# JacobYoung115/VisualSLAM

Hardware: AMD Instinct MI355X
Metric: frames/sec @1080p (Harris + DoG keypoint detection) (higher is better)
Workload: dtype u8

## Files before the change

### visualslam_amd/csrc/diff_taps.gen.h

```cpp
#pragma once
#include <cstdint>

namespace vslam {
namespace dtaps {

constexpr int OCT_LO = 1, OCT_HI = 3;

template <int O, int L>
struct Lvl;

template <>
struct Lvl<1, 0> {
    static constexpr int n = 19, form = 0, nd = 18;
    static constexpr uint16_t w[n] = {1, 1, 3, 6, 9, 15, 20, 27, 30, 32, 30, 27, 20, 15, 9, 6, 3, 1, 1};
    static constexpr int16_t de[nd] = {-10, -8, -7, -6, -5, -4, -3, -2, -1, 0, 1, 2, 3, 4, 5, 6, 7, 9};
    static constexpr int16_t dc[nd] = {-1, -2, -3, -3, -6, -5, -7, -3, -2, 2, 3, 7, 5, 6, 3, 3, 2, 1};
};

template <>
struct Lvl<1, 1> {
    static constexpr int n = 23, form = 0, nd = 22;
    static constexpr uint16_t w[n] = {1, 1, 2, 4, 5, 9, 12, 15, 19, 23, 24, 26, 24, 23, 19, 15, 12, 9, 5, 4, 2, 1, 1};
    static constexpr int16_t de[nd] = {-12, -10, -9, -8, -7, -6, -5, -4, -3, -2, -1, 0, 1, 2, 3, 4, 5, 6, 7, 8, 9, 11};
    static constexpr int16_t dc[nd] = {-1, -1, -2, -1, -4, -3, -3, -4, -4, -1, -2, 2, 1, 4, 4, 3, 3, 4, 1, 2, 1, 1};
};

template <>
struct Lvl<1, 2> {
    static constexpr int n = 29, form = 0, nd = 26;
    static constexpr uint16_t w[n] = {1, 0, 2, 2, 3, 4, 6, 7, 10, 13, 15, 17, 18, 20, 20, 20, 18, 17, 15, 13, 10, 7, 6, 4, 3, 2, 2, 0, 1};
    static constexpr int16_t de[nd] = {-15, -14, -13, -11, -10, -9, -8, -7, -6, -5, -4, -3, -2, 1, 2, 3, 4, 5, 6, 7, 8, 9, 10, 12, 13, 14};
    static constexpr int16_t dc[nd] = {-1, 1, -2, -1, -1, -2, -1, -3, -3, -2, -2, -1, -2, 2, 1, 2, 2, 3, 3, 1, 2, 1, 1, 2, -1, 1};
};

template <>
struct Lvl<1, 3> {
    static constexpr int n = 37, form = 1, nd = 24;
    static constexpr uint16_t w[n] = {1, 0, 1, 1, 1, 2, 3, 4, 4, 6, 8, 8, 11, 11, 14, 14, 15, 16, 16, 16, 15, 14, 14, 11, 11, 8, 8, 6, 4, 4, 3, 2, 1, 1, 1, 0, 1};
    static constexpr int16_t de[nd] = {-19, -18, -17, -14, -13, -12, -10, -9, -7, -5, -3, -2, 1, 2, 4, 6, 8, 9, 11, 12, 13, 16, 17, 18};
    static constexpr int16_t dc[nd] = {-1, 1, -1, -1, -1, -1, -2, -2, -3, -3, -1, -1, 1, 1, 3, 3, 2, 2, 1, 1, 1, 1, -1, 1};
};

template <>
struct Lvl<1, 4> {
    static constexpr int n = 45, form = 1, nd = 36;
    static constexpr uint16_t w[n] = {1, 0, 1, 0, 2, 1, 2, 2, 3, 3, 4, 5, 6, 7, 8, 9, 9, 11, 11, 12, 12, 13, 12, 13, 12, 12, 11, 11, 9, 9, 8, 7, 6, 5, 4, 3, 3, 2, 2, 1, 2, 0, 1, 0, 1};
    static constexpr int16_t de[nd] = {-23, -22, -21, -20, -19, -18, -17, -15, -13, -12, -11, -10, -9, -8, -6, -4, -2, -1, 0, 1, 3, 5, 7, 8, 9, 10, 11, 12, 14, 16, 17, 18, 19, 20, 21, 22};
    static constexpr int16_t dc[nd] = {-1, 1, -1, 1, -2, 1, -1, -1, -1, -1, -1, -1, -1, -1, -2, -1, -1, 1, -1, 1, 1, 2, 1, 1, 1, 1, 1, 1, 1, 1, -1, 2, -1, 1, -1, 1};
};

template <>
struct Lvl<1, 5> {
    static constexpr int n = 57, form = 1, nd = 28;
    static constexpr uint16_t w[n] = {1, 0, 0, 1, 0, 1, 1, 1, 2, 2, 2, 2, 3, 3, 4, 5, 5, 5, 7, 6, 8, 8, 8, 9, 9, 10, 10, 10, 10, 10, 10, 10, 9, 9, 8, 8, 8, 6, 7, 5, 5, 5, 4, 3, 3, 2, 2, 2, 2, 1, 1, 1, 0, 1, 0, 0, 1};
    static constexpr int16_t de[nd] = {-29, -28, -26, -25, -24, -21, -17, -15, -14, -11, -10, -9, -6, -4, 3, 5, 8, 9, 10, 13, 14, 16, 20, 23, 24, 25, 27, 28};
    static constexpr int16_t dc[nd] = {-1, 1, -1, 1, -1, -1, -1, -1, -1, -2, 1, -2, -1, -1, 1, 1, 2, -1, 2, 1, 1, 1, 1, 1, -1, 1, -1, 1};
};

template <>
struct Lvl<2, 0> {
    static constexpr int n = 37, form = 1, nd = 24;
    static constexpr uint16_t w[n] = {1, 0, 1, 1, 1, 2, 3, 4, 4, 6, 8, 8, 11, 11, 14, 14, 15, 16, 16, 16, 15, 14, 14, 11, 11, 8, 8, 6, 4, 4, 3, 2, 1, 1, 1, 0, 1};
    static constexpr int16_t de[nd] = {-19, -18, -17, -14, -13, -12, -10, -9, -7, -5, -3, -2, 1, 2, 4, 6, 8, 9, 11, 12, 13, 16, 17, 18};
    static constexpr int16_t dc[nd] = {-1, 1, -1, -1, -1, -1, -2, -2, -3, -3, -1, -1, 1, 1, 3, 3, 2, 2, 1, 1, 1, 1, -1, 1};
};

template <>
struct Lvl<2, 1> {
    static constexpr int n = 45, form = 1, nd = 36;
    static constexpr uint16_t w[n] = {1, 0, 1, 0, 2, 1, 2, 2, 3, 3, 4, 5, 6, 7, 8, 9, 9, 11, 11, 12, 12, 13, 12, 13, 12, 12, 11, 11, 9, 9, 8, 7, 6, 5, 4, 3, 3, 2, 2, 1, 2, 0, 1, 0, 1};
    static constexpr int16_t de[nd] = {-23, -22, -21, -20, -19, -18, -17, -15, -13, -12, -11, -10, -9, -8, -6, -4, -2, -1, 0, 1, 3, 5, 7, 8, 9, 10, 11, 12, 14, 16, 17, 18, 19, 20, 21, 22};
    static constexpr int16_t dc[nd] = {-1, 1, -1, 1, -2, 1, -1, -1, -1, -1, -1, -1, -1, -1, -2, -1, -1, 1, -1, 1, 1, 2, 1, 1, 1, 1, 1, 1, 1, 1, -1, 2, -1, 1, -1, 1};
};

template <>
struct Lvl<2, 2> {
    static constexpr int n = 57, form = 1, nd = 28;
    static constexpr uint16_t w[n] = {1, 0, 0, 1, 0, 1, 1, 1, 2, 2, 2, 2, 3, 3, 4, 5, 5, 5, 7, 6, 8, 8, 8, 9, 9, 10, 10, 10, 10, 10, 10, 10, 9, 9, 8, 8, 8, 6, 7, 5, 5, 5, 4, 3, 3, 2, 2, 2, 2, 1, 1, 1, 0, 1, 0, 0, 1};
    static constexpr int16_t de[nd] = {-29, -28, -26, -25, -24, -21, -17, -15, -14, -11, -10, -9, -6, -4, 3, 5, 8, 9, 10, 13, 14, 16, 20, 23, 24, 25, 27, 28};
    static constexpr int16_t dc[nd] = {-1, 1, -1, 1, -1, -1, -1, -1, -1, -2, 1, -2, -1, -1, 1, 1, 2, -1, 2, 1, 1, 1, 1, 1, -1, 1, -1, 1};
};

template <>
struct Lvl<2, 3> {
    static constexpr int n = 71, form = 1, nd = 34;
    static constexpr uint16_t w[n] = {1, 0, 0, 1, 0, 0, 1, 1, 1, 1, 1, 1, 2, 2, 2, 2, 3, 3, 3, 4, 4, 4, 5, 5, 6, 5, 7, 6, 7, 7, 8, 7, 8, 8, 8, 8, 8, 8, 8, 7, 8, 7, 7, 6, 7, 5, 6, 5, 5, 4, 4, 4, 3, 3, 3, 2, 2, 2, 2, 1, 1, 1, 1, 1, 1, 0, 0, 1, 0, 0, 1};
    static constexpr int16_t de[nd] = {-36, -35, -33, -32, -30, -24, -20, -17, -14, -12, -11, -10, -9, -8, -6, -5, -4, 3, 4, 5, 7, 8, 9, 10, 11, 13, 16, 19, 23, 29, 31, 32, 34, 35};
    static constexpr int16_t dc[nd] = {-1, 1, -1, 1, -1, -1, -1, -1, -1, -1, 1, -2, 1, -1, -1, 1, -1, 1, -1, 1, 1, -1, 2, -1, 1, 1, 1, 1, 1, 1, -1, 1, -1, 1};
};

template <>
struct Lvl<2, 4> {
    static constexpr int n = 89, form = 1, nd = 44;
    static constexpr uint16_t w[n] = {1, 0, 0, 0, 1, 0, 0, 1, 0, 1, 1, 0, 1, 1, 1, 2, 1, 2, 1, 2, 2, 3, 2, 3, 3, 3, 3, 4, 4, 4, 4, 5, 5, 5, 5, 5, 6, 6, 6, 6, 6, 6, 6, 7, 6, 7, 6, 6, 6, 6, 6, 6, 6, 5, 5, 5, 5, 5, 4, 4, 4, 4, 3, 3, 3, 3, 2, 3, 2, 2, 1, 2, 1, 2, 1, 1, 1, 0, 1, 1, 0, 1, 0, 0, 1, 0, 0, 0, 1};
    static constexpr int16_t de[nd] = {-45, -44, -41, -40, -38, -37, -36, -34, -33, -30, -29, -28, -27, -26, -24, -23, -22, -18, -14, -9, -2, -1, 0, 1, 8, 13, 17, 21, 22, 23, 25, 26, 27, 28, 29, 32, 33, 35, 36, 37, 39, 40, 43, 44};
    static constexpr int16_t dc[nd] = {-1, 1, -1, 1, -1, 1, -1, 1, -1, -1, 1, -1, 1, -1, -1, 1, -1, -1, -1, -1, -1, 1, -1, 1, 1, 1, 1, 1, -1, 1, 1, -1, 1, -1, 1, 1, -1, 1, -1, 1, -1, 1, -1, 1};
};

template <>
struct Lvl<2, 5> {
    static constexpr int n = 111, form = 1, nd = 56;
    static constexpr uint16_t w[n] = {1, 0, 0, 0, 0, 1, 0, 0, 1, 0, 0, 1, 0, 1, 1, 0, 1, 1, 1, 1, 1, 1, 2, 1, 2, 1, 2, 2, 2, 3, 2, 2, 3, 3, 3, 3, 3, 4, 3, 4, 4, 4, 4, 4, 4, 5, 4, 5, 5, 5, 5, 4, 5, 5, 5, 6, 5, 5, 5, 4, 5, 5, 5, 5, 4, 5, 4, 4, 4, 4, 4, 4, 3, 4, 3, 3, 3, 3, 3, 2, 2, 3, 2, 2, 2, 1, 2, 1, 2, 1, 1, 1, 1, 1, 1, 0, 1, 1, 0, 1, 0, 0, 1, 0, 0, 1, 0, 0, 0, 0, 1};
    static constexpr int16_t de[nd] = {-56, -55, -51, -50, -48, -47, -45, -44, -43, -41, -40, -34, -33, -32, -31, -30, -27, -26, -24, -19, -18, -17, -11, -10, -9, -5, -4, -1, 0, 3, 4, 8, 9, 10, 16, 17, 18, 23, 25, 26, 29, 30, 31, 32, 33, 39, 40, 42, 43, 44, 46, 47, 49, 50, 54, 55};
    static constexpr int16_t dc[nd] = {-1, 1, -1, 1, -1, 1, -1, 1, -1, 1, -1, -1, 1, -1, 1, -1, -1, 1, -1, -1, 1, -1, -1, 1, -1, 1, -1, -1, 1, 1, -1, 1, -1, 1, 1, -1, 1, 1, -1, 1, 1, -1, 1, -1, 1, 1, -1, 1, -1, 1, -1, 1, -1, 1, -1, 1};
};

template <>
struct Lvl<3, 0> {
    static constexpr int n = 71, form = 1, nd = 34;
    static constexpr uint16_t w[n] = {1, 0, 0, 1, 0, 0, 1, 1, 1, 1, 1, 1, 2, 2, 2, 2, 3, 3, 3, 4, 4, 4, 5, 5, 6, 5, 7, 6, 7, 7, 8, 7, 8, 8, 8, 8, 8, 8, 8, 7, 8, 7, 7, 6, 7, 5, 6, 5, 5, 4, 4, 4, 3, 3, 3, 2, 2, 2, 2, 1, 1, 1, 1, 1, 1, 0, 0, 1, 0, 0, 1};
    static constexpr int16_t de[nd] = {-36, -35, -33, -32, -30, -24, -20, -17, -14, -12, -11, -10, -9, -8, -6, -5, -4, 3, 4, 5, 7, 8, 9, 10, 11, 13, 16, 19, 23, 29, 31, 32, 34, 35};
    static constexpr int16_t dc[nd] = {-1, 1, -1, 1, -1, -1, -1, -1, -1, -1, 1, -2, 1, -1, -1, 1, -1, 1, -1, 1, 1, -1, 2, -1, 1, 1, 1, 1, 1, 1, -1, 1, -1, 1};
};

template <>
struct Lvl<3, 1> {
    static constexpr int n = 89, form = 1, nd = 44;
    static constexpr uint16_t w[n] = {1, 0, 0, 0, 1, 0, 0, 1, 0, 1, 1, 0, 1, 1, 1, 2, 1, 2, 1, 2, 2, 3, 2, 3, 3, 3, 3, 4, 4, 4, 4, 5, 5, 5, 5, 5, 6, 6, 6, 6, 6, 6, 6, 7, 6, 7, 6, 6, 6, 6, 6, 6, 6, 5, 5, 5, 5, 5, 4, 4, 4, 4, 3, 3, 3, 3, 2, 3, 2, 2, 1, 2, 1, 2, 1, 1, 1, 0, 1, 1, 0, 1, 0, 0, 1, 0, 0, 0, 1};
    static constexpr int16_t de[nd] = {-45, -44, -41, -40, -38, -37, -36, -34, -33, -30, -29, -28, -27, -26, -24, -23, -22, -18, -14, -9, -2, -1, 0, 1, 8, 13, 17, 21, 22, 23, 25, 26, 27, 28, 29, 32, 33, 35, 36, 37, 39, 40, 43, 44};
    static constexpr int16_t dc[nd] = {-1, 1, -1, 1, -1, 1, -1, 1, -1, -1, 1, -1, 1, -1, -1, 1, -1, -1, -1, -1, -1, 1, -1, 1, 1, 1, 1, 1, -1, 1, 1, -1, 1, -1, 1, 1, -1, 1, -1, 1, -1, 1, -1, 1};
};

template <>
struct Lvl<3, 2> {
    static constexpr int n = 111, form = 1, nd = 56;
    static constexpr uint16_t w[n] = {1, 0, 0, 0, 0, 1, 0, 0, 1, 0, 0, 1, 0, 1, 1, 0, 1, 1, 1, 1, 1, 1, 2, 1, 2, 1, 2, 2, 2, 3, 2, 2, 3, 3, 3, 3, 3, 4, 3, 4, 4, 4, 4, 4, 4, 5, 4, 5, 5, 5, 5, 4, 5, 5, 5, 6, 5, 5, 5, 4, 5, 5, 5, 5, 4, 5, 4, 4, 4, 4, 4, 4, 3, 4, 3, 3, 3, 3, 3, 2, 2, 3, 2, 2, 2, 1, 2, 1, 2, 1, 1, 1, 1, 1, 1, 0, 1, 1, 0, 1, 0, 0, 1, 0, 0, 1, 0, 0, 0, 0, 1};
    static constexpr int16_t de[nd] = {-56, -55, -51, -50, -48, -47, -45, -44, -43, -41, -40, -34, -33, -32, -31, -30, -27, -26, -24, -19, -18, -17, -11, -10, -9, -5, -4, -1, 0, 3, 4, 8, 9, 10, 16, 17, 18, 23, 25, 26, 29, 30, 31, 32, 33, 39, 40, 42, 43, 44, 46, 47, 49, 50, 54, 55};
    static constexpr int16_t dc[nd] = {-1, 1, -1, 1, -1, 1, -1, 1, -1, 1, -1, -1, 1, -1, 1, -1, -1, 1, -1, -1, 1, -1, -1, 1, -1, 1, -1, -1, 1, 1, -1, 1, -1, 1, 1, -1, 1, 1, -1, 1, 1, -1, 1, -1, 1, 1, -1, 1, -1, 1, -1, 1, -1, 1, -1, 1};
};

template <>
struct Lvl<3, 3> {
    static constexpr int n = 141, form = 1, nd = 64;
    static constexpr uint16_t w[n] = {1, 0, 0, 0, 0, 0, 0, 1, 0, 0, 0, 1, 0, 0, 1, 0, 0, 1, 0, 1, 1, 0, 1, 1, 0, 1, 1, 1, 1, 1, 1, 2, 1, 1, 2, 1, 2, 2, 2, 2, 2, 2, 2, 2, 3, 2, 3, 2, 3, 3, 3, 3, 3, 3, 4, 3, 3, 4, 4, 3, 4, 4, 3, 4, 4, 4, 4, 4, 4, 4, 4, 4, 4, 4, 4, 4, 4, 4, 3, 4, 4, 3, 4, 4, 3, 3, 4, 3, 3, 3, 3, 3, 3, 2, 3, 2, 3, 2, 2, 2, 2, 2, 2, 2, 2, 1, 2, 1, 1, 2, 1, 1, 1, 1, 1, 1, 0, 1, 1, 0, 1, 1, 0, 1, 0, 0, 1, 0, 0, 1, 0, 0, 0, 1, 0, 0, 0, 0, 0, 0, 1};
    static constexpr int16_t de[nd] = {-71, -70, -64, -63, -60, -59, -57, -56, -54, -53, -52, -50, -49, -47, -46, -40, -39, -37, -36, -35, -27, -26, -25, -24, -23, -17, -16, -14, -12, -11, -9, -8, 7, 8, 10, 11, 13, 15, 16, 22, 23, 24, 25, 26, 34, 35, 36, 38, 39, 45, 46, 48, 49, 51, 52, 53, 55, 56, 58, 59, 62, 63, 69, 70};
    static constexpr int16_t dc[nd] = {-1, 1, -1, 1, -1, 1, -1, 1, -1, 1, -1, 1, -1, 1, -1, -1, 1, -1, 1, -1, -1, 1, -1, 1, -1, -1, 1, -1, 1, -1, 1, -1, 1, -1, 1, -1, 1, -1, 1, 1, -1, 1, -1, 1, 1, -1, 1, -1, 1, 1, -1, 1, -1, 1, -1, 1, -1, 1, -1, 1, -1, 1, -1, 1};
};

template <>
struct Lvl<3, 4> {
    static constexpr int n = 177, form = 1, nd = 80;
    static constexpr uint16_t w[n] = {1, 0, 0, 0, 0, 0, 0, 0, 0, 1, 0, 0, 0, 0, 1, 0, 0, 0, 1, 0, 0, 1, 0, 1, 0, 0, 1, 0, 1, 1, 0, 1, 1, 0, 1, 1, 1, 1, 1, 1, 1, 1, 1, 1, 1, 2, 1, 2, 1, 2, 1, 2, 1, 2, 2, 2, 2, 2, 2, 2, 2, 2, 3, 2, 3, 2, 2, 3, 3, 2, 3, 3, 3, 2, 3, 3, 3, 3, 3, 3, 3, 4, 3, 3, 3, 3, 3, 3, 4, 3, 3, 3, 3, 3, 3, 4, 3, 3, 3, 3, 3, 3, 3, 2, 3, 3, 3, 2, 3, 3, 2, 2, 3, 2, 3, 2, 2, 2, 2, 2, 2, 2, 2, 2, 1, 2, 1, 2, 1, 2, 1, 2, 1, 1, 1, 1, 1, 1, 1, 1, 1, 1, 1, 0, 1, 1, 0, 1, 1, 0, 1, 0, 0, 1, 0, 1, 0, 0, 1, 0, 0, 0, 1, 0, 0, 0, 0, 1, 0, 0, 0, 0, 0, 0, 0, 0, 1};
    static constexpr int16_t de[nd] = {-89, -88, -80, -79, -75, -74, -71, -70, -68, -67, -66, -65, -63, -62, -61, -59, -58, -56, -55, -44, -43, -42, -41, -40, -39, -38, -37, -36, -27, -26, -25, -24, -22, -20, -19, -16, -15, -8, -7, -1, 0, 6, 7, 14, 15, 18, 19, 21, 23, 24, 25, 26, 35, 36, 37, 38, 39, 40, 41, 42, 43, 54, 55, 57, 58, 60, 61, 62, 64, 65, 66, 67, 69, 70, 73, 74, 78, 79, 87, 88};
    static constexpr int16_t dc[nd] = {-1, 1, -1, 1, -1, 1, -1, 1, -1, 1, -1, 1, -1, 1, -1, 1, -1, 1, -1, -1, 1, -1, 1, -1, 1, -1, 1, -1, -1, 1, -1, 1, -1, 1, -1, 1, -1, -1, 1, -1, 1, -1, 1, 1, -1, 1, -1, 1, -1, 1, -1, 1, 1, -1, 1, -1, 1, -1, 1, -1, 1, 1, -1, 1, -1, 1, -1, 1, -1, 1, -1, 1, -1, 1, -1, 1, -1, 1, -1, 1};
};

template <>
struct Lvl<3, 5> {
    static constexpr int n = 223, form = 1, nd = 116;
    static constexpr uint16_t w[n] = {1, 0, 0, 0, 0, 0, 0, 0, 0, 0, 0, 1, 0, 0, 0, 0, 0, 0, 1, 0, 0, 0, 0, 1, 0, 0, 0, 1, 0, 0, 1, 0, 1, 0, 0, 1, 0, 1, 0, 1, 0, 1, 0, 1, 1, 0, 1, 1, 1, 0, 1, 1, 1, 1, 1, 1, 1, 1, 1, 1, 1, 1, 2, 1, 1, 1, 2, 1, 2, 1, 2, 1, 2, 1, 2, 2, 1, 2, 2, 2, 2, 2, 2, 2, 2, 2, 2, 2, 2, 2, 2, 3, 2, 2, 3, 2, 2, 3, 2, 2, 3, 2, 3, 2, 3, 2, 3, 2, 3, 2, 3, 2, 3, 2, 3, 2, 3, 2, 3, 2, 3, 2, 3, 2, 2, 3, 2, 2, 3, 2, 2, 3, 2, 2, 2, 2, 2, 2, 2, 2, 2, 2, 2, 2, 2, 2, 1, 2, 2, 1, 2, 1, 2, 1, 2, 1, 2, 1, 1, 1, 2, 1, 1, 1, 1, 1, 1, 1, 1, 1, 1, 1, 1, 0, 1, 1, 1, 0, 1, 1, 0, 1, 0, 1, 0, 1, 0, 1, 0, 0, 1, 0, 1, 0, 0, 1, 0, 0, 0, 1, 0, 0, 0, 0, 1, 0, 0, 0, 0, 0, 0, 1, 0, 0, 0, 0, 0, 0, 0, 0, 0, 0, 1};
    static constexpr int16_t de[nd] = {-112, -111, -101, -100, -94, -93, -89, -88, -85, -84, -82, -81, -80, -79, -77, -76, -75, -74, -73, -72, -71, -70, -69, -67, -66, -63, -62, -50, -49, -46, -45, -44, -43, -42, -41, -40, -39, -38, -36, -35, -21, -20, -18, -17, -15, -14, -12, -11, -10, -9, -8, -7, -6, -5, -4, -3, -2, -1, 0, 1, 2, 3, 4, 5, 6, 7, 8, 9, 10, 11, 13, 14, 16, 17, 19, 20, 34, 35, 37, 38, 39, 40, 41, 42, 43, 44, 45, 48, 49, 61, 62, 65, 66, 68, 69, 70, 71, 72, 73, 74, 75, 76, 78, 79, 80, 81, 83, 84, 87, 88, 92, 93, 99, 100, 110, 111};
    static constexpr int16_t dc[nd] = {-1, 1, -1, 1, -1, 1, -1, 1, -1, 1, -1, 1, -1, 1, -1, 1, -1, 1, -1, 1, -1, 1, -1, 1, -1, 1, -1, -1, 1, -1, 1, -1, 1, -1, 1, -1, 1, -1, 1, -1, -1, 1, -1, 1, -1, 1, -1, 1, -1, 1, -1, 1, -1, 1, -1, 1, -1, 1, -1, 1, -1, 1, -1, 1, -1, 1, -1, 1, -1, 1, -1, 1, -1, 1, -1, 1, 1, -1, 1, -1, 1, -1, 1, -1, 1, -1, 1, -1, 1, 1, -1, 1, -1, 1, -1, 1, -1, 1, -1, 1, -1, 1, -1, 1, -1, 1, -1, 1, -1, 1, -1, 1, -1, 1, -1, 1};
};

}
}
```

### visualslam_amd/csrc/kernels_hdiff.hip.h

```cpp
#pragma once
#include <hip/hip_runtime.h>

#include <utility>
#include <vector>

#include "diff_taps.gen.h"
#include "kernels_strip.hip.h"
#include "vslam_internal.h"

namespace vslam {

constexpr int HD_J = 16;
constexpr int HD_PAD = 2;

typedef float hd_f2 __attribute__((ext_vector_type(2)));

template <class F, int... I>
__device__ __forceinline__ void hd_for_impl(F&& f, std::integer_sequence<int, I...>) {
    (f(std::integral_constant<int, I>{}), ...);
}
template <int N, class F>
__device__ __forceinline__ void hd_for(F&& f) {
    hd_for_impl(f, std::make_integer_sequence<int, N>{});
}

__host__ __device__ constexpr int hd_phys(int c) { return c + (c >> 4) * HD_PAD; }

template <class LV>
__host__ __device__ constexpr int hd_w(int k) { return k >= 0 && k < LV::n ? (int)LV::w[k] : 0; }

template <class LV>
__host__ __device__ constexpr int hd_coef(int e) {
    if (LV::form == 1) {
        for (int i = 0; i < LV::nd; ++i)
            if (LV::de[i] == e) return LV::dc[i];
        return 0;
    }
    return hd_w<LV>(e + LV::n / 2);
}

template <int O>
struct HdGeom {
    static constexpr int nmax = dtaps::Lvl<O, 5>::n;
    static constexpr int rmax = nmax / 2;
    static constexpr int HL = (rmax + 2 + 15) & ~15;
    static_assert(dtaps::Lvl<O, 0>::n <= nmax && dtaps::Lvl<O, 4>::n <= nmax, "level 5 is the widest");
};

__host__ __device__ inline int hd_pw(int cols, int HL, int rmax) {
    const int ccount = HL + 16 * ((cols + HD_J - 1) / HD_J) + rmax;
    return (ccount + 1 + 15) / 16 * (16 + HD_PAD);
}

template <class LV, int HL>
__device__ __forceinline__ void hd_level(const hd_f2* __restrict__ lane, hd_f2 (&acc)[HD_J]) {
    constexpr int n = LV::n, r = n / 2;
    constexpr bool DIFF = LV::form == 1;
    constexpr int lo = DIFF ? -r - 1 : -r, hi = HD_J - 1 + r;
    constexpr int t0 = (HL + lo) & ~1, Q = (HL + hi - t0) / 2 + 1;
    hd_f2 seed = {0.f, 0.f};
    hd_for<HD_J>([&](auto j) { acc[decltype(j)::value] = hd_f2{0.f, 0.f}; });
    hd_for<Q>([&](auto q) {
        constexpr int t = t0 + 2 * decltype(q)::value;
        const float4 v = *reinterpret_cast<const float4*>(lane + hd_phys(t));
        const hd_f2 hv[2] = {hd_f2{v.x, v.y}, hd_f2{v.z, v.w}};
        hd_for<2>([&](auto b) {
            constexpr int x = t + decltype(b)::value - HL;
            if constexpr (DIFF) {
                constexpr int wk = hd_w<LV>(x + 1 + r);
                if constexpr (wk != 0) seed = __builtin_elementwise_fma(hd_f2((float)wk), hv[decltype(b)::value], seed);
            }
            hd_for<HD_J>([&](auto j) {
                constexpr int c = hd_coef<LV>(x - decltype(j)::value);
                if constexpr (c != 0)
                    acc[decltype(j)::value] = __builtin_elementwise_fma(hd_f2((float)c), hv[decltype(b)::value], acc[decltype(j)::value]);
            });
        });
    });
    if constexpr (DIFF) {
        acc[0] += seed;
        hd_for<HD_J - 1>([&](auto j) { acc[decltype(j)::value + 1] += acc[decltype(j)::value]; });
    }
}

template <int O>
__global__ __launch_bounds__(256) void k_gauss_h_diff(const uint16_t* __restrict__ h, size_t hframe, uint8_t* __restrict__ oct_out,
                                                       size_t pframe, int rows, int cols, int pitch, int npairs, int pw,
                                                       uint8_t* __restrict__ next_base, size_t nframe, int nrows, int ncols, int npitch) {
    using G = HdGeom<O>;
    extern __shared__ __attribute__((aligned(16))) uint32_t smem[];
    hd_f2* hp = reinterpret_cast<hd_f2*>(smem);
    const int tid = threadIdx.x;
    const int y0 = blockIdx.y * 2 * npairs;
    const size_t P = (size_t)rows * pitch;
    uint8_t* out = oct_out + blockIdx.z * pframe;
    const int ncs = (cols + HD_J - 1) / HD_J;
    const int ccount = G::HL + HD_J * ncs + G::rmax;
    const int n8 = cols >> 3, nb = ccount - 8 * n8;
    const bool active = tid < npairs * ncs;
    const int ip = tid / ncs, is = tid - ip * ncs;
    const hd_f2* lane = hp + ip * pw + is * (HD_J + HD_PAD);
    const int n8d = max(n8, 1);
    const int i_p0 = tid / n8d, i_k0 = tid - i_p0 * n8d, i_dp = 256 / n8d, i_dk = 256 - i_dp * n8d;
    const int b_p0 = tid / nb, b_i0 = tid - b_p0 * nb, b_dp = 256 / nb, b_di = 256 - b_dp * nb;
    uint32_t prev_e[2][4], prev_o[2][4];

    hd_for<VSLAM_NUM_LEVELS>([&](auto lc) {
        constexpr int L = decltype(lc)::value;
        const uint16_t* hl = h + blockIdx.z * hframe + (size_t)L * P;
        __syncthreads();
        for (int it = tid, p = i_p0, k = i_k0; it < npairs * n8; it += 256, p += i_dp, k += i_dk) {
            if (k >= n8) k -= n8, ++p;
            const uint4 a = *reinterpret_cast<const uint4*>(hl + (size_t)min(y0 + 2 * p, rows - 1) * pitch + 8 * k);
            const uint4 b = *reinterpret_cast<const uint4*>(hl + (size_t)min(y0 + 2 * p + 1, rows - 1) * pitch + 8 * k);
            float4* q = reinterpret_cast<float4*>(hp + p * pw + hd_phys(G::HL + 8 * k));
            const uint32_t av[4] = {a.x, a.y, a.z, a.w}, bv[4] = {b.x, b.y, b.z, b.w};
#pragma unroll
            for (int i = 0; i < 4; ++i)
                q[i] = make_float4((float)(av[i] & 0xffffu), (float)(bv[i] & 0xffffu), (float)(av[i] >> 16), (float)(bv[i] >> 16));
        }
        for (int it = tid, p = b_p0, i = b_i0; it < npairs * nb; it += 256, p += b_dp, i += b_di) {
            if (i >= nb) i -= nb, ++p;
            const int c = i < G::HL ? i : 8 * n8 + i;
            const int x = reflect101(c - G::HL, cols);
            const uint16_t* ra = hl + (size_t)min(y0 + 2 * p, rows - 1) * pitch;
            const uint16_t* rb = hl + (size_t)min(y0 + 2 * p + 1, rows - 1) * pitch;
            hp[p * pw + hd_phys(c)] = hd_f2{(float)ra[x], (float)rb[x]};
        }
        __syncthreads();
        if (active) {
            hd_f2 acc[HD_J];
            hd_level<dtaps::Lvl<O, L>, G::HL>(lane, acc);
            const int x = HD_J * is;
            hd_for<2>([&](auto rc) {
                constexpr int rho = decltype(rc)::value;
                const int y = y0 + 2 * ip + rho;
                uint32_t u[HD_J], g[4], d[4];
                hd_for<HD_J>([&](auto j) { u[decltype(j)::value] = (uint32_t)acc[decltype(j)::value][rho]; });
#pragma unroll
                for (int hw = 0; hw < 4; ++hw) {
                    const uint32_t e = __builtin_amdgcn_perm(u[4 * hw + 2], u[4 * hw + 0], 0x0c060c02);
                    const uint32_t o = __builtin_amdgcn_perm(u[4 * hw + 3], u[4 * hw + 1], 0x0c060c02);
                    g[hw] = __builtin_amdgcn_perm(o, e, 0x06020400);
                    if constexpr (L > 0)
                        d[hw] = __builtin_amdgcn_perm(pk_sub_sat_u16(o, prev_o[rho][hw]), pk_sub_sat_u16(e, prev_e[rho][hw]), 0x06020400);
                    prev_e[rho][hw] = e;
                    prev_o[rho][hw] = o;
                }
                if (y < rows) {
                    const size_t off = (size_t)y * pitch + x;
                    *reinterpret_cast<uint4*>(out + (size_t)L * P + off) = make_uint4(g[0], g[1], g[2], g[3]);
                    if constexpr (L > 0)
                        *reinterpret_cast<uint4*>(out + (size_t)(VSLAM_NUM_LEVELS + L - 1) * P + off) = make_uint4(d[0], d[1], d[2], d[3]);
                    if constexpr (L == 3 && rho == 0)
                        if (next_base && (y >> 1) < nrows && (x >> 1) < ncols)
                            *reinterpret_cast<uint2*>(next_base + blockIdx.z * nframe + (size_t)(y >> 1) * npitch + (x >> 1)) =
                                make_uint2(__builtin_amdgcn_perm(g[1], g[0], 0x06040200), __builtin_amdgcn_perm(g[3], g[2], 0x06040200));
                }
            });
        }
    });
}

template <int O, int L>
static bool hd_level_matches(const std::vector<uint16_t>& t) {
    using LV = dtaps::Lvl<O, L>;
    if ((int)t.size() != LV::n) return false;
    for (int k = 0; k < LV::n; ++k)
        if (t[k] != LV::w[k]) return false;
    std::vector<int> off, coef;
    if (diff_form(t.data(), LV::n, off, coef) != LV::form) return false;
    if (LV::form == 1) {
        if ((int)off.size() != LV::nd) return false;
        for (int i = 0; i < LV::nd; ++i)
            if (off[i] != LV::de[i] || coef[i] != LV::dc[i]) return false;
    }
    return true;
}
template <int O>
static bool hd_octave_matches(const std::vector<uint16_t> (&taps)[6]) {
    return hd_level_matches<O, 0>(taps[0]) && hd_level_matches<O, 1>(taps[1]) && hd_level_matches<O, 2>(taps[2]) &&
           hd_level_matches<O, 3>(taps[3]) && hd_level_matches<O, 4>(taps[4]) && hd_level_matches<O, 5>(taps[5]);
}

}
```

### visualslam_amd/csrc/vslam_internal.h

```cpp
#pragma once
#include <cstddef>
#include <cstdint>
#include <vector>

#include "../../include/vslam.h"

#define VSLAM_MAX_KSIZE 4095

namespace vslam {
int gauss_ksize_u8(double sigma);
bool gauss_taps_q8(int n, double sigma, uint16_t* taps);
bool gauss_taps_q8_trimmed(int n, double sigma, std::vector<uint16_t>& out);
int gauss_ksize_f32(double sigma);
bool gauss_kernel_f32(int n, double sigma, std::vector<float>& out);
double sigma_at(double sigma0, int octave, int level);
int auto_num_octaves(int rows, int cols);
void half_size(int rows, int cols, int* r, int* c);
void extrema_lattice(int rows, int cols, int window, int* lr, int* lc);
int make_layout(const vslam_params* p, vslam_batch_layout* L);
int diff_form(const uint16_t* w, int n, std::vector<int>& off, std::vector<int>& coef);
}

extern "C" int vslam_diff_form_q8(const uint16_t* taps, int n, int* offsets, int* coeffs, int cap, int* nnz);
```

### visualslam_amd/csrc/vslam_params.cpp

```cpp
#include <cmath>
#include <cstdio>
#include <cstring>
#include <vector>

#include "../../include/vslam.h"
#include "vslam_internal.h"

namespace vslam {

static inline long cv_round(double v) { return std::lrint(v); }

int gauss_ksize_u8(double sigma) { return (int)cv_round(sigma * 3 * 2 + 1) | 1; }

static void gauss_kernel_f64(int n, double sigma, std::vector<double>& kf) {
    kf.assign((size_t)n, 0.0);
    const int half = (n - 1) / 2;
    static const double k3[] = {0.25, 0.5, 0.25};
    static const double k5[] = {0.0625, 0.25, 0.375, 0.25, 0.0625};
    static const double k7[] = {0.03125, 0.109375, 0.21875, 0.28125, 0.21875, 0.109375, 0.03125};
    if (sigma <= 0 && n == 1) {
        kf[0] = 1.0;
    } else if (sigma <= 0 && n == 3) {
        kf.assign(k3, k3 + 3);
    } else if (sigma <= 0 && n == 5) {
        kf.assign(k5, k5 + 5);
    } else if (sigma <= 0 && n == 7) {
        kf.assign(k7, k7 + 7);
    } else {
        const double s = sigma > 0 ? sigma : std::fma((double)n, 0.15, 0.35);
        const double scale = -0.125 / (s * s);
        double sum = 0.0;
        for (int i = 0, x = 1 - n; i < half; ++i, x += 2) {
            kf[i] = std::exp((double)(x * x) * scale);
            sum += kf[i];
        }
        sum = sum * 2.0 + 1.0;
        const double inv = 1.0 / sum;
        for (int i = 0; i < half; ++i) kf[n - 1 - i] = kf[i] = kf[i] * inv;
        kf[half] = inv;
    }
}

int gauss_ksize_f32(double sigma) { return (int)cv_round(sigma * 4 * 2 + 1) | 1; }

bool gauss_kernel_f32(int n, double sigma, std::vector<float>& out) {
    if (n <= 0 || (n & 1) == 0 || n > (1 << 20)) return false;
    std::vector<double> kf;
    gauss_kernel_f64(n, sigma, kf);
    out.resize((size_t)n);
    for (int i = 0; i < n; ++i) out[(size_t)i] = (float)kf[(size_t)i];
    return true;
}

bool gauss_taps_q8(int n, double sigma, uint16_t* taps) {
    if (n <= 0 || (n & 1) == 0 || n > VSLAM_MAX_KSIZE) return false;
    std::vector<double> kf;
    gauss_kernel_f64(n, sigma, kf);
    double err = 0.0;
    long acc = 0;
    for (int i = 0; i < n / 2; ++i) {
        const double adj = kf[i] * 256.0 + err;
        const long q = cv_round(adj);
        err = adj - (double)q;
        taps[i] = taps[n - 1 - i] = (uint16_t)q;
        acc += q;
    }
    taps[n / 2] = (uint16_t)(256 - 2 * acc);
    return true;
}

bool gauss_taps_q8_trimmed(int n, double sigma, std::vector<uint16_t>& out) {
    std::vector<uint16_t> t((size_t)(n > 0 ? n : 0));
    if (!gauss_taps_q8(n, sigma, t.data())) return false;
    int z = 0;
    while (2 * z + 1 < n && t[z] == 0 && t[n - 1 - z] == 0) ++z;
    out.assign(t.begin() + z, t.end() - z);
    return true;
}

static constexpr long DIFF_HMAX = 255 * 256 + 128;

int diff_form(const uint16_t* w, int n, std::vector<int>& off, std::vector<int>& coef) {
    off.clear(), coef.clear();
    if (!w || n <= 0 || (n & 1) == 0) return -1;
    const int r = n / 2;
    long l1 = 0;
    for (int e = -r - 1; e <= r; ++e) {
        const int k = e + r;
        const int d = (k >= 0 ? (int)w[k] : 0) - (k + 1 < n ? (int)w[k + 1] : 0);
        if (d) off.push_back(e), coef.push_back(d), l1 += d < 0 ? -d : d;
    }
    if (l1 * DIFF_HMAX >= (1L << 24)) return 0;
    return (double)off.size() * 2.32 * 1.15 <= (double)(n + 1) / 2 * 4.27 ? 1 : 0;
}

double sigma_at(double sigma0, int octave, int level) {
    const double k = std::pow(2.0f, 1.0f / (double)3);
    return std::pow(2, octave) * sigma0 * std::pow(k, level);
}

int auto_num_octaves(int rows, int cols) {
    const int m = rows < cols ? rows : cols;
    return (int)std::floor(std::log2((double)m)) - 4;
}

void half_size(int rows, int cols, int* r, int* c) {
    *r = (int)cv_round(rows * 0.5);
    *c = (int)cv_round(cols * 0.5);
}

void extrema_lattice(int rows, int cols, int window, int* lr, int* lc) {
    const int pad = (window - 1) / 2;
    *lr = rows > pad ? (rows - pad + window - 1) / window : 0;
    *lc = cols > pad ? (cols - pad + window - 1) / window : 0;
}

int make_layout(const vslam_params* p, vslam_batch_layout* L) {
    if (!p || !L || p->rows <= 0 || p->cols <= 0 || p->n_octaves < 0 || p->n_octaves > VSLAM_MAX_OCTAVES)
        return VSLAM_ERR_INVALID;
    if (p->n_octaves > 0 && (!(p->sigma0 > 0) || p->extrema_window < 3 || (p->extrema_window & 1) == 0))
        return VSLAM_ERR_INVALID;
    if (p->n_octaves > 0 && p->extrema_dense && (p->extrema_window != 3 || p->localize || p->orient)) return VSLAM_ERR_INVALID;
    std::memset(L, 0, sizeof(*L));
    L->n_octaves = p->n_octaves;
    int r = p->rows * 2, c = p->cols * 2;
    size_t off = 0, woff = 0, sum_p = 0;
    for (int o = 0; o < p->n_octaves; ++o) {
        if (r <= 0 || c <= 0) return VSLAM_ERR_INVALID;
        L->rows[o] = r;
        L->cols[o] = c;
        if (p->extrema_dense)
            L->lat_rows[o] = r, L->lat_cols[o] = c;
        else
            extrema_lattice(r, c, p->extrema_window, &L->lat_rows[o], &L->lat_cols[o]);
        L->lat_words[o] = (L->lat_cols[o] + 63) / 64;
        L->octave_offset[o] = off;
        L->bits_offset[o] = woff;
        L->pitch[o] = (c + 15) & ~15;
        const size_t P = (size_t)r * c;
        sum_p += P;
        off += (VSLAM_NUM_LEVELS + VSLAM_NUM_DOGS) * ((size_t)r * L->pitch[o]);
        woff += (size_t)3 * L->lat_rows[o] * L->lat_words[o];
        half_size(r, c, &r, &c);
    }
    L->pyramid_frame_bytes = (off + 255) & ~(size_t)255;
    L->bits_frame_words = woff;
    const size_t N = (size_t)p->rows * p->cols;
    L->algorithmic_bytes_harris = 6 * N;
    L->algorithmic_bytes_dog = N + 11 * sum_p;
    return VSLAM_OK;
}

}

extern "C" {

int vslam_version(void) { return VSLAM_VERSION; }

const char* vslam_status_string(int s) {
    switch (s) {
        case VSLAM_OK: return "ok";
        case VSLAM_ERR_INVALID: return "invalid argument";
        case VSLAM_ERR_HIP: return "HIP runtime error";
        case VSLAM_ERR_NOMEM: return "out of memory";
        case VSLAM_ERR_UNSUPPORTED: return "unsupported parameter combination";
        case VSLAM_ERR_RANGE: return "octave/level out of range";
        default: return "unknown status";
    }
}

int vslam_gauss_ksize_u8(double sigma) { return vslam::gauss_ksize_u8(sigma); }

int vslam_gauss_taps_q8(int n, double sigma, uint16_t* taps) {
    if (!taps) return VSLAM_ERR_INVALID;
    return vslam::gauss_taps_q8(n, sigma, taps) ? VSLAM_OK : VSLAM_ERR_INVALID;
}

double vslam_sigma_at(double sigma0, int octave, int level) { return vslam::sigma_at(sigma0, octave, level); }

int vslam_diff_form_q8(const uint16_t* taps, int n, int* offsets, int* coeffs, int cap, int* nnz) {
    std::vector<int> off, coef;
    const int form = vslam::diff_form(taps, n, off, coef);
    if (form < 0 || !nnz || (int)off.size() > cap || (!off.empty() && (!offsets || !coeffs))) return -1;
    *nnz = (int)off.size();
    for (size_t i = 0; i < off.size(); ++i) offsets[i] = off[i], coeffs[i] = coef[i];
    return form;
}
int vslam_auto_num_octaves(int rows, int cols) { return vslam::auto_num_octaves(rows, cols); }

void vslam_half_size(int rows, int cols, int* out_rows, int* out_cols) {
    vslam::half_size(rows, cols, out_rows, out_cols);
}

void vslam_extrema_lattice(int rows, int cols, int window, int* lat_rows, int* lat_cols) {
    vslam::extrema_lattice(rows, cols, window, lat_rows, lat_cols);
}

void vslam_params_default(vslam_params* p, int rows, int cols) {
    if (!p) return;
    p->rows = rows;
    p->cols = cols;
    p->n_octaves = 4;
    p->sigma0 = 1.6;
    p->harris_k = 0.04f;
    p->do_harris = 1;
    p->extrema_window = 3;
    p->min_contrast = 8;
    p->localize = 0;
    p->orient = 0;
    p->extrema_dense = 0;
    const unsigned long long N = rows > 0 && cols > 0 ? (unsigned long long)rows * (unsigned long long)cols : 0ull;
    auto cap_of = [](unsigned long long v, unsigned long long lo) {
        v = (v + 4095ull) & ~4095ull;
        return (uint32_t)(v < lo ? lo : v > 0x40000000ull ? 0x40000000ull : v);
    };
    p->oriented_cap = cap_of(N / 32, 1ull << 14);
    p->harris_cap = cap_of(N / 8, 1ull << 16);
    p->dog_cap = cap_of(N / 8, 1ull << 16);
}

int vslam_batch_out_required(const vslam_params* p, int n_frames, vslam_batch_out* z) {
    vslam_batch_layout L;
    if (!z || n_frames <= 0 || vslam::make_layout(p, &L) != VSLAM_OK) return VSLAM_ERR_INVALID;
    const size_t n = (size_t)n_frames, N = (size_t)p->rows * p->cols;
    z->struct_size = sizeof(vslam_batch_out);
    z->response_bytes = n * N * sizeof(float);
    z->nms_mask_bytes = n * N;
    z->nms2_bytes = n * N * sizeof(float);
    z->harris_kps_bytes = n * p->harris_cap * sizeof(vslam_kp);
    z->harris_counts_bytes = n * sizeof(uint32_t);
    z->pyramid_bytes = n * L.pyramid_frame_bytes;
    z->extrema_bits_bytes = n * L.bits_frame_words * sizeof(uint64_t);
    z->dog_points_bytes = n * p->dog_cap * sizeof(vslam_point);
    z->dog_counts_bytes = n * sizeof(uint32_t);
    z->oriented_points_bytes = n * p->oriented_cap * sizeof(vslam_point);
    z->oriented_counts_bytes = n * sizeof(uint32_t);
    z->oriented_survivors_bytes = n * sizeof(uint32_t);
    z->descriptors_bytes = n * p->oriented_cap * 128 * sizeof(float);
    z->descriptor_defined_bytes = n * p->oriented_cap;
    return VSLAM_OK;
}

int vslam_batch_layout_query(const vslam_params* p, vslam_batch_layout* out) { return vslam::make_layout(p, out); }

void vslam_cos_sin_deg(float theta_deg, float* c, float* s) {
    const float angle = (float)((double)theta_deg * (3.1415926535897932384626433832795 / (double)180.0f));
    if (c) *c = (float)std::cos((double)angle);
    if (s) *s = (float)std::sin((double)angle);
}

int vslam_rotated_window_points(int cx, int cy, int window, float theta_deg, int32_t* xy) {
    if (!xy || window <= 0) return VSLAM_ERR_INVALID;
    float c, s;
    vslam_cos_sin_deg(theta_deg, &c, &s);
    const int padding = window / 2;
    int q = 0;
    for (int i = cy - padding; i <= cy + padding; ++i)
        for (int j = cx - padding; j <= cx + padding; ++j, ++q) {
            const int rx = j - cx, ry = i - cy;
            const float a = (float)rx * c, b = (float)ry * s, d = (float)rx * s, e = (float)ry * c;
            xy[2 * q] = (int)(a - b) + cx;
            xy[2 * q + 1] = (int)(d + e) + cy;
        }
    return VSLAM_OK;
}

int vslam_descriptor_file_write(const char* path, const float* desc, size_t n) {
    if (!path || (!desc && n) || n > 0x7fffffff) return VSLAM_ERR_INVALID;
    std::FILE* f = std::fopen(path, "wb");
    if (!f) return VSLAM_ERR_INVALID;
    const int32_t head[3] = {(int32_t)n, 128, 24};
    bool ok = std::fwrite(head, sizeof(int32_t), 3, f) == 3;
    if (n) ok = ok && std::fwrite(desc, sizeof(float) * 128, n, f) == n;
    ok = (std::fclose(f) == 0) && ok;
    return ok ? VSLAM_OK : VSLAM_ERR_INVALID;
}

void vslam_points16_expand(const vslam_point16* in, size_t n, vslam_point* out) {
    if (!in || !out) return;
    for (size_t i = 0; i < n; ++i) {
        const uint32_t t = in[i].tag;
        out[i].row = in[i].row, out[i].col = in[i].col, out[i].value = in[i].value;
        out[i].padding = (int32_t)(t >> 16), out[i].octave = (int32_t)((t >> 8) & 0xffu), out[i].level = (int32_t)(t & 0xffu);
    }
}

}
```

Measured before the change: 14870.

## Split Gaussian taps into smooth step part plus sparse spikes to cut FMAs

```diff
diff --git a/visualslam_amd/csrc/diff_taps.gen.h b/visualslam_amd/csrc/diff_taps.gen.h
--- a/visualslam_amd/csrc/diff_taps.gen.h
+++ b/visualslam_amd/csrc/diff_taps.gen.h
@@ -15,6 +15,11 @@
     static constexpr uint16_t w[n] = {1, 1, 3, 6, 9, 15, 20, 27, 30, 32, 30, 27, 20, 15, 9, 6, 3, 1, 1};
     static constexpr int16_t de[nd] = {-10, -8, -7, -6, -5, -4, -3, -2, -1, 0, 1, 2, 3, 4, 5, 6, 7, 9};
     static constexpr int16_t dc[nd] = {-1, -2, -3, -3, -6, -5, -7, -3, -2, 2, 3, 7, 5, 6, 3, 3, 2, 1};
+    static constexpr int mixed = 0, ns = 16, nb = 1;
+    static constexpr int16_t se[16] = {-10, -8, -7, -6, -5, -4, -3, -2, 1, 2, 3, 4, 5, 6, 7, 9};
+    static constexpr int16_t sc[16] = {-1, -2, -3, -3, -6, -5, -7, -3, 3, 7, 5, 6, 3, 3, 2, 1};
+    static constexpr int16_t be[1] = {0};
+    static constexpr int16_t bc[1] = {2};
 };
 
 template <>
@@ -23,6 +28,11 @@
     static constexpr uint16_t w[n] = {1, 1, 2, 4, 5, 9, 12, 15, 19, 23, 24, 26, 24, 23, 19, 15, 12, 9, 5, 4, 2, 1, 1};
     static constexpr int16_t de[nd] = {-12, -10, -9, -8, -7, -6, -5, -4, -3, -2, -1, 0, 1, 2, 3, 4, 5, 6, 7, 8, 9, 11};
     static constexpr int16_t dc[nd] = {-1, -1, -2, -1, -4, -3, -3, -4, -4, -1, -2, 2, 1, 4, 4, 3, 3, 4, 1, 2, 1, 1};
+    static constexpr int mixed = 0, ns = 20, nb = 1;
+    static constexpr int16_t se[20] = {-12, -10, -9, -8, -7, -6, -5, -4, -3, -2, 1, 2, 3, 4, 5, 6, 7, 8, 9, 11};
+    static constexpr int16_t sc[20] = {-1, -1, -2, -1, -4, -3, -3, -4, -4, -1, 1, 4, 4, 3, 3, 4, 1, 2, 1, 1};
+    static constexpr int16_t be[1] = {0};
+    static constexpr int16_t bc[1] = {2};
 };
 
 template <>
@@ -31,6 +41,11 @@
     static constexpr uint16_t w[n] = {1, 0, 2, 2, 3, 4, 6, 7, 10, 13, 15, 17, 18, 20, 20, 20, 18, 17, 15, 13, 10, 7, 6, 4, 3, 2, 2, 0, 1};
     static constexpr int16_t de[nd] = {-15, -14, -13, -11, -10, -9, -8, -7, -6, -5, -4, -3, -2, 1, 2, 3, 4, 5, 6, 7, 8, 9, 10, 12, 13, 14};
     static constexpr int16_t dc[nd] = {-1, 1, -2, -1, -1, -2, -1, -3, -3, -2, -2, -1, -2, 2, 1, 2, 2, 3, 3, 1, 2, 1, 1, 2, -1, 1};
+    static constexpr int mixed = 0, ns = 22, nb = 2;
+    static constexpr int16_t se[22] = {-13, -11, -10, -9, -8, -7, -6, -5, -4, -3, -2, 1, 2, 3, 4, 5, 6, 7, 8, 9, 10, 12};
+    static constexpr int16_t sc[22] = {-2, -1, -1, -2, -1, -3, -3, -2, -2, -1, -2, 2, 1, 2, 2, 3, 3, 1, 2, 1, 1, 2};
+    static constexpr int16_t be[2] = {-14, 14};
+    static constexpr int16_t bc[2] = {1, 1};
 };
 
 template <>
@@ -39,6 +54,11 @@
     static constexpr uint16_t w[n] = {1, 0, 1, 1, 1, 2, 3, 4, 4, 6, 8, 8, 11, 11, 14, 14, 15, 16, 16, 16, 15, 14, 14, 11, 11, 8, 8, 6, 4, 4, 3, 2, 1, 1, 1, 0, 1};
     static constexpr int16_t de[nd] = {-19, -18, -17, -14, -13, -12, -10, -9, -7, -5, -3, -2, 1, 2, 4, 6, 8, 9, 11, 12, 13, 16, 17, 18};
     static constexpr int16_t dc[nd] = {-1, 1, -1, -1, -1, -1, -2, -2, -3, -3, -1, -1, 1, 1, 3, 3, 2, 2, 1, 1, 1, 1, -1, 1};
+    static constexpr int mixed = 1, ns = 20, nb = 2;
+    static constexpr int16_t se[20] = {-17, -14, -13, -12, -10, -9, -7, -5, -3, -2, 1, 2, 4, 6, 8, 9, 11, 12, 13, 16};
+    static constexpr int16_t sc[20] = {-1, -1, -1, -1, -2, -2, -3, -3, -1, -1, 1, 1, 3, 3, 2, 2, 1, 1, 1, 1};
+    static constexpr int16_t be[2] = {-18, 18};
+    static constexpr int16_t bc[2] = {1, 1};
 };
 
 template <>
@@ -47,6 +67,11 @@
     static constexpr uint16_t w[n] = {1, 0, 1, 0, 2, 1, 2, 2, 3, 3, 4, 5, 6, 7, 8, 9, 9, 11, 11, 12, 12, 13, 12, 13, 12, 12, 11, 11, 9, 9, 8, 7, 6, 5, 4, 3, 3, 2, 2, 1, 2, 0, 1, 0, 1};
     static constexpr int16_t de[nd] = {-23, -22, -21, -20, -19, -18, -17, -15, -13, -12, -11, -10, -9, -8, -6, -4, -2, -1, 0, 1, 3, 5, 7, 8, 9, 10, 11, 12, 14, 16, 17, 18, 19, 20, 21, 22};
     static constexpr int16_t dc[nd] = {-1, 1, -1, 1, -2, 1, -1, -1, -1, -1, -1, -1, -1, -1, -2, -1, -1, 1, -1, 1, 1, 2, 1, 1, 1, 1, 1, 1, 1, 1, -1, 2, -1, 1, -1, 1};
+    static constexpr int mixed = 1, ns = 20, nb = 8;
+    static constexpr int16_t se[20] = {-19, -15, -13, -12, -11, -10, -9, -8, -6, -4, 3, 5, 7, 8, 9, 10, 11, 12, 14, 18};
+    static constexpr int16_t sc[20] = {-2, -1, -1, -1, -1, -1, -1, -1, -2, -1, 1, 2, 1, 1, 1, 1, 1, 1, 1, 2};
+    static constexpr int16_t be[8] = {-22, -20, -17, -1, 1, 17, 20, 22};
+    static constexpr int16_t bc[8] = {1, 1, -1, 1, 1, -1, 1, 1};
 };
 
 template <>
@@ -55,6 +80,11 @@
     static constexpr uint16_t w[n] = {1, 0, 0, 1, 0, 1, 1, 1, 2, 2, 2, 2, 3, 3, 4, 5, 5, 5, 7, 6, 8, 8, 8, 9, 9, 10, 10, 10, 10, 10, 10, 10, 9, 9, 8, 8, 8, 6, 7, 5, 5, 5, 4, 3, 3, 2, 2, 2, 2, 1, 1, 1, 0, 1, 0, 0, 1};
     static constexpr int16_t de[nd] = {-29, -28, -26, -25, -24, -21, -17, -15, -14, -11, -10, -9, -6, -4, 3, 5, 8, 9, 10, 13, 14, 16, 20, 23, 24, 25, 27, 28};
     static constexpr int16_t dc[nd] = {-1, 1, -1, 1, -1, -1, -1, -1, -1, -2, 1, -2, -1, -1, 1, 1, 2, -1, 2, 1, 1, 1, 1, 1, -1, 1, -1, 1};
+    static constexpr int mixed = 1, ns = 20, nb = 4;
+    static constexpr int16_t se[20] = {-24, -21, -17, -15, -14, -11, -10, -9, -6, -4, 3, 5, 8, 9, 10, 13, 14, 16, 20, 23};
+    static constexpr int16_t sc[20] = {-1, -1, -1, -1, -1, -2, 1, -2, -1, -1, 1, 1, 2, -1, 2, 1, 1, 1, 1, 1};
+    static constexpr int16_t be[4] = {-28, -25, 25, 28};
+    static constexpr int16_t bc[4] = {1, 1, 1, 1};
 };
 
 template <>
@@ -63,6 +93,11 @@
     static constexpr uint16_t w[n] = {1, 0, 1, 1, 1, 2, 3, 4, 4, 6, 8, 8, 11, 11, 14, 14, 15, 16, 16, 16, 15, 14, 14, 11, 11, 8, 8, 6, 4, 4, 3, 2, 1, 1, 1, 0, 1};
     static constexpr int16_t de[nd] = {-19, -18, -17, -14, -13, -12, -10, -9, -7, -5, -3, -2, 1, 2, 4, 6, 8, 9, 11, 12, 13, 16, 17, 18};
     static constexpr int16_t dc[nd] = {-1, 1, -1, -1, -1, -1, -2, -2, -3, -3, -1, -1, 1, 1, 3, 3, 2, 2, 1, 1, 1, 1, -1, 1};
+    static constexpr int mixed = 1, ns = 20, nb = 2;
+    static constexpr int16_t se[20] = {-17, -14, -13, -12, -10, -9, -7, -5, -3, -2, 1, 2, 4, 6, 8, 9, 11, 12, 13, 16};
+    static constexpr int16_t sc[20] = {-1, -1, -1, -1, -2, -2, -3, -3, -1, -1, 1, 1, 3, 3, 2, 2, 1, 1, 1, 1};
+    static constexpr int16_t be[2] = {-18, 18};
+    static constexpr int16_t bc[2] = {1, 1};
 };
 
 template <>
@@ -71,6 +106,11 @@
     static constexpr uint16_t w[n] = {1, 0, 1, 0, 2, 1, 2, 2, 3, 3, 4, 5, 6, 7, 8, 9, 9, 11, 11, 12, 12, 13, 12, 13, 12, 12, 11, 11, 9, 9, 8, 7, 6, 5, 4, 3, 3, 2, 2, 1, 2, 0, 1, 0, 1};
     static constexpr int16_t de[nd] = {-23, -22, -21, -20, -19, -18, -17, -15, -13, -12, -11, -10, -9, -8, -6, -4, -2, -1, 0, 1, 3, 5, 7, 8, 9, 10, 11, 12, 14, 16, 17, 18, 19, 20, 21, 22};
     static constexpr int16_t dc[nd] = {-1, 1, -1, 1, -2, 1, -1, -1, -1, -1, -1, -1, -1, -1, -2, -1, -1, 1, -1, 1, 1, 2, 1, 1, 1, 1, 1, 1, 1, 1, -1, 2, -1, 1, -1, 1};
+    static constexpr int mixed = 1, ns = 20, nb = 8;
+    static constexpr int16_t se[20] = {-19, -15, -13, -12, -11, -10, -9, -8, -6, -4, 3, 5, 7, 8, 9, 10, 11, 12, 14, 18};
+    static constexpr int16_t sc[20] = {-2, -1, -1, -1, -1, -1, -1, -1, -2, -1, 1, 2, 1, 1, 1, 1, 1, 1, 1, 2};
+    static constexpr int16_t be[8] = {-22, -20, -17, -1, 1, 17, 20, 22};
+    static constexpr int16_t bc[8] = {1, 1, -1, 1, 1, -1, 1, 1};
 };
 
 template <>
@@ -79,6 +119,11 @@
     static constexpr uint16_t w[n] = {1, 0, 0, 1, 0, 1, 1, 1, 2, 2, 2, 2, 3, 3, 4, 5, 5, 5, 7, 6, 8, 8, 8, 9, 9, 10, 10, 10, 10, 10, 10, 10, 9, 9, 8, 8, 8, 6, 7, 5, 5, 5, 4, 3, 3, 2, 2, 2, 2, 1, 1, 1, 0, 1, 0, 0, 1};
     static constexpr int16_t de[nd] = {-29, -28, -26, -25, -24, -21, -17, -15, -14, -11, -10, -9, -6, -4, 3, 5, 8, 9, 10, 13, 14, 16, 20, 23, 24, 25, 27, 28};
     static constexpr int16_t dc[nd] = {-1, 1, -1, 1, -1, -1, -1, -1, -1, -2, 1, -2, -1, -1, 1, 1, 2, -1, 2, 1, 1, 1, 1, 1, -1, 1, -1, 1};
+    static constexpr int mixed = 1, ns = 20, nb = 4;
+    static constexpr int16_t se[20] = {-24, -21, -17, -15, -14, -11, -10, -9, -6, -4, 3, 5, 8, 9, 10, 13, 14, 16, 20, 23};
+    static constexpr int16_t sc[20] = {-1, -1, -1, -1, -1, -2, 1, -2, -1, -1, 1, 1, 2, -1, 2, 1, 1, 1, 1, 1};
+    static constexpr int16_t be[4] = {-28, -25, 25, 28};
+    static constexpr int16_t bc[4] = {1, 1, 1, 1};
 };
 
 template <>
@@ -87,6 +132,11 @@
     static constexpr uint16_t w[n] = {1, 0, 0, 1, 0, 0, 1, 1, 1, 1, 1, 1, 2, 2, 2, 2, 3, 3, 3, 4, 4, 4, 5, 5, 6, 5, 7, 6, 7, 7, 8, 7, 8, 8, 8, 8, 8, 8, 8, 7, 8, 7, 7, 6, 7, 5, 6, 5, 5, 4, 4, 4, 3, 3, 3, 2, 2, 2, 2, 1, 1, 1, 1, 1, 1, 0, 0, 1, 0, 0, 1};
     static constexpr int16_t de[nd] = {-36, -35, -33, -32, -30, -24, -20, -17, -14, -12, -11, -10, -9, -8, -6, -5, -4, 3, 4, 5, 7, 8, 9, 10, 11, 13, 16, 19, 23, 29, 31, 32, 34, 35};
     static constexpr int16_t dc[nd] = {-1, 1, -1, 1, -1, -1, -1, -1, -1, -1, 1, -2, 1, -1, -1, 1, -1, 1, -1, 1, 1, -1, 2, -1, 1, 1, 1, 1, 1, 1, -1, 1, -1, 1};
+    static constexpr int mixed = 1, ns = 14, nb = 10;
+    static constexpr int16_t se[14] = {-30, -24, -20, -17, -14, -10, -4, 3, 9, 13, 16, 19, 23, 29};
+    static constexpr int16_t sc[14] = {-1, -1, -1, -1, -1, -2, -1, 1, 2, 1, 1, 1, 1, 1};
+    static constexpr int16_t be[10] = {-35, -32, -11, -8, -5, 5, 8, 11, 32, 35};
+    static constexpr int16_t bc[10] = {1, 1, 1, -1, 1, 1, -1, 1, 1, 1};
 };
 
 template <>
@@ -95,6 +145,11 @@
     static constexpr uint16_t w[n] = {1, 0, 0, 0, 1, 0, 0, 1, 0, 1, 1, 0, 1, 1, 1, 2, 1, 2, 1, 2, 2, 3, 2, 3, 3, 3, 3, 4, 4, 4, 4, 5, 5, 5, 5, 5, 6, 6, 6, 6, 6, 6, 6, 7, 6, 7, 6, 6, 6, 6, 6, 6, 6, 5, 5, 5, 5, 5, 4, 4, 4, 4, 3, 3, 3, 3, 2, 3, 2, 2, 1, 2, 1, 2, 1, 1, 1, 0, 1, 1, 0, 1, 0, 0, 1, 0, 0, 0, 1};
     static constexpr int16_t de[nd] = {-45, -44, -41, -40, -38, -37, -36, -34, -33, -30, -29, -28, -27, -26, -24, -23, -22, -18, -14, -9, -2, -1, 0, 1, 8, 13, 17, 21, 22, 23, 25, 26, 27, 28, 29, 32, 33, 35, 36, 37, 39, 40, 43, 44};
     static constexpr int16_t dc[nd] = {-1, 1, -1, 1, -1, 1, -1, 1, -1, -1, 1, -1, 1, -1, -1, 1, -1, -1, -1, -1, -1, 1, -1, 1, 1, 1, 1, 1, -1, 1, 1, -1, 1, -1, 1, 1, -1, 1, -1, 1, -1, 1, -1, 1};
+    static constexpr int mixed = 1, ns = 12, nb = 16;
+    static constexpr int16_t se[12] = {-36, -26, -22, -18, -14, -9, 8, 13, 17, 21, 25, 35};
+    static constexpr int16_t sc[12] = {-1, -1, -1, -1, -1, -1, 1, 1, 1, 1, 1, 1};
+    static constexpr int16_t be[16] = {-44, -40, -37, -33, -29, -27, -23, -1, 1, 23, 27, 29, 33, 37, 40, 44};
+    static constexpr int16_t bc[16] = {1, 1, 1, -1, 1, 1, 1, 1, 1, 1, 1, 1, -1, 1, 1, 1};
 };
 
 template <>
@@ -103,6 +158,11 @@
     static constexpr uint16_t w[n] = {1, 0, 0, 0, 0, 1, 0, 0, 1, 0, 0, 1, 0, 1, 1, 0, 1, 1, 1, 1, 1, 1, 2, 1, 2, 1, 2, 2, 2, 3, 2, 2, 3, 3, 3, 3, 3, 4, 3, 4, 4, 4, 4, 4, 4, 5, 4, 5, 5, 5, 5, 4, 5, 5, 5, 6, 5, 5, 5, 4, 5, 5, 5, 5, 4, 5, 4, 4, 4, 4, 4, 4, 3, 4, 3, 3, 3, 3, 3, 2, 2, 3, 2, 2, 2, 1, 2, 1, 2, 1, 1, 1, 1, 1, 1, 0, 1, 1, 0, 1, 0, 0, 1, 0, 0, 1, 0, 0, 0, 0, 1};
     static constexpr int16_t de[nd] = {-56, -55, -51, -50, -48, -47, -45, -44, -43, -41, -40, -34, -33, -32, -31, -30, -27, -26, -24, -19, -18, -17, -11, -10, -9, -5, -4, -1, 0, 3, 4, 8, 9, 10, 16, 17, 18, 23, 25, 26, 29, 30, 31, 32, 33, 39, 40, 42, 43, 44, 46, 47, 49, 50, 54, 55};
     static constexpr int16_t dc[nd] = {-1, 1, -1, 1, -1, 1, -1, 1, -1, 1, -1, -1, 1, -1, 1, -1, -1, 1, -1, -1, 1, -1, -1, 1, -1, 1, -1, -1, 1, 1, -1, 1, -1, 1, 1, -1, 1, 1, -1, 1, 1, -1, 1, -1, 1, 1, -1, 1, -1, 1, -1, 1, -1, 1, -1, 1};
+    static constexpr int mixed = 1, ns = 10, nb = 23;
+    static constexpr int16_t se[10] = {-43, -30, -24, -17, -9, 8, 16, 23, 29, 42};
+    static constexpr int16_t sc[10] = {-1, -1, -1, -1, -1, 1, 1, 1, 1, 1};
+    static constexpr int16_t be[23] = {-55, -50, -47, -44, -40, -33, -31, -26, -18, -10, -4, 0, 4, 10, 18, 26, 31, 33, 40, 44, 47, 50, 55};
+    static constexpr int16_t bc[23] = {1, 1, 1, 1, -1, 1, 1, 1, 1, 1, -1, 1, -1, 1, 1, 1, 1, 1, -1, 1, 1, 1, 1};
 };
 
 template <>
@@ -111,6 +171,11 @@
     static constexpr uint16_t w[n] = {1, 0, 0, 1, 0, 0, 1, 1, 1, 1, 1, 1, 2, 2, 2, 2, 3, 3, 3, 4, 4, 4, 5, 5, 6, 5, 7, 6, 7, 7, 8, 7, 8, 8, 8, 8, 8, 8, 8, 7, 8, 7, 7, 6, 7, 5, 6, 5, 5, 4, 4, 4, 3, 3, 3, 2, 2, 2, 2, 1, 1, 1, 1, 1, 1, 0, 0, 1, 0, 0, 1};
     static constexpr int16_t de[nd] = {-36, -35, -33, -32, -30, -24, -20, -17, -14, -12, -11, -10, -9, -8, -6, -5, -4, 3, 4, 5, 7, 8, 9, 10, 11, 13, 16, 19, 23, 29, 31, 32, 34, 35};
     static constexpr int16_t dc[nd] = {-1, 1, -1, 1, -1, -1, -1, -1, -1, -1, 1, -2, 1, -1, -1, 1, -1, 1, -1, 1, 1, -1, 2, -1, 1, 1, 1, 1, 1, 1, -1, 1, -1, 1};
+    static constexpr int mixed = 1, ns = 14, nb = 10;
+    static constexpr int16_t se[14] = {-30, -24, -20, -17, -14, -10, -4, 3, 9, 13, 16, 19, 23, 29};
+    static constexpr int16_t sc[14] = {-1, -1, -1, -1, -1, -2, -1, 1, 2, 1, 1, 1, 1, 1};
+    static constexpr int16_t be[10] = {-35, -32, -11, -8, -5, 5, 8, 11, 32, 35};
+    static constexpr int16_t bc[10] = {1, 1, 1, -1, 1, 1, -1, 1, 1, 1};
 };
 
 template <>
@@ -119,6 +184,11 @@
     static constexpr uint16_t w[n] = {1, 0, 0, 0, 1, 0, 0, 1, 0, 1, 1, 0, 1, 1, 1, 2, 1, 2, 1, 2, 2, 3, 2, 3, 3, 3, 3, 4, 4, 4, 4, 5, 5, 5, 5, 5, 6, 6, 6, 6, 6, 6, 6, 7, 6, 7, 6, 6, 6, 6, 6, 6, 6, 5, 5, 5, 5, 5, 4, 4, 4, 4, 3, 3, 3, 3, 2, 3, 2, 2, 1, 2, 1, 2, 1, 1, 1, 0, 1, 1, 0, 1, 0, 0, 1, 0, 0, 0, 1};
     static constexpr int16_t de[nd] = {-45, -44, -41, -40, -38, -37, -36, -34, -33, -30, -29, -28, -27, -26, -24, -23, -22, -18, -14, -9, -2, -1, 0, 1, 8, 13, 17, 21, 22, 23, 25, 26, 27, 28, 29, 32, 33, 35, 36, 37, 39, 40, 43, 44};
     static constexpr int16_t dc[nd] = {-1, 1, -1, 1, -1, 1, -1, 1, -1, -1, 1, -1, 1, -1, -1, 1, -1, -1, -1, -1, -1, 1, -1, 1, 1, 1, 1, 1, -1, 1, 1, -1, 1, -1, 1, 1, -1, 1, -1, 1, -1, 1, -1, 1};
+    static constexpr int mixed = 1, ns = 12, nb = 16;
+    static constexpr int16_t se[12] = {-36, -26, -22, -18, -14, -9, 8, 13, 17, 21, 25, 35};
+    static constexpr int16_t sc[12] = {-1, -1, -1, -1, -1, -1, 1, 1, 1, 1, 1, 1};
+    static constexpr int16_t be[16] = {-44, -40, -37, -33, -29, -27, -23, -1, 1, 23, 27, 29, 33, 37, 40, 44};
+    static constexpr int16_t bc[16] = {1, 1, 1, -1, 1, 1, 1, 1, 1, 1, 1, 1, -1, 1, 1, 1};
 };
 
 template <>
@@ -127,6 +197,11 @@
     static constexpr uint16_t w[n] = {1, 0, 0, 0, 0, 1, 0, 0, 1, 0, 0, 1, 0, 1, 1, 0, 1, 1, 1, 1, 1, 1, 2, 1, 2, 1, 2, 2, 2, 3, 2, 2, 3, 3, 3, 3, 3, 4, 3, 4, 4, 4, 4, 4, 4, 5, 4, 5, 5, 5, 5, 4, 5, 5, 5, 6, 5, 5, 5, 4, 5, 5, 5, 5, 4, 5, 4, 4, 4, 4, 4, 4, 3, 4, 3, 3, 3, 3, 3, 2, 2, 3, 2, 2, 2, 1, 2, 1, 2, 1, 1, 1, 1, 1, 1, 0, 1, 1, 0, 1, 0, 0, 1, 0, 0, 1, 0, 0, 0, 0, 1};
     static constexpr int16_t de[nd] = {-56, -55, -51, -50, -48, -47, -45, -44, -43, -41, -40, -34, -33, -32, -31, -30, -27, -26, -24, -19, -18, -17, -11, -10, -9, -5, -4, -1, 0, 3, 4, 8, 9, 10, 16, 17, 18, 23, 25, 26, 29, 30, 31, 32, 33, 39, 40, 42, 43, 44, 46, 47, 49, 50, 54, 55};
     static constexpr int16_t dc[nd] = {-1, 1, -1, 1, -1, 1, -1, 1, -1, 1, -1, -1, 1, -1, 1, -1, -1, 1, -1, -1, 1, -1, -1, 1, -1, 1, -1, -1, 1, 1, -1, 1, -1, 1, 1, -1, 1, 1, -1, 1, 1, -1, 1, -1, 1, 1, -1, 1, -1, 1, -1, 1, -1, 1, -1, 1};
+    static constexpr int mixed = 1, ns = 10, nb = 23;
+    static constexpr int16_t se[10] = {-43, -30, -24, -17, -9, 8, 16, 23, 29, 42};
+    static constexpr int16_t sc[10] = {-1, -1, -1, -1, -1, 1, 1, 1, 1, 1};
+    static constexpr int16_t be[23] = {-55, -50, -47, -44, -40, -33, -31, -26, -18, -10, -4, 0, 4, 10, 18, 26, 31, 33, 40, 44, 47, 50, 55};
+    static constexpr int16_t bc[23] = {1, 1, 1, 1, -1, 1, 1, 1, 1, 1, -1, 1, -1, 1, 1, 1, 1, 1, -1, 1, 1, 1, 1};
 };
 
 template <>
@@ -135,6 +210,11 @@
     static constexpr uint16_t w[n] = {1, 0, 0, 0, 0, 0, 0, 1, 0, 0, 0, 1, 0, 0, 1, 0, 0, 1, 0, 1, 1, 0, 1, 1, 0, 1, 1, 1, 1, 1, 1, 2, 1, 1, 2, 1, 2, 2, 2, 2, 2, 2, 2, 2, 3, 2, 3, 2, 3, 3, 3, 3, 3, 3, 4, 3, 3, 4, 4, 3, 4, 4, 3, 4, 4, 4, 4, 4, 4, 4, 4, 4, 4, 4, 4, 4, 4, 4, 3, 4, 4, 3, 4, 4, 3, 3, 4, 3, 3, 3, 3, 3, 3, 2, 3, 2, 3, 2, 2, 2, 2, 2, 2, 2, 2, 1, 2, 1, 1, 2, 1, 1, 1, 1, 1, 1, 0, 1, 1, 0, 1, 1, 0, 1, 0, 0, 1, 0, 0, 1, 0, 0, 0, 1, 0, 0, 0, 0, 0, 0, 1};
     static constexpr int16_t de[nd] = {-71, -70, -64, -63, -60, -59, -57, -56, -54, -53, -52, -50, -49, -47, -46, -40, -39, -37, -36, -35, -27, -26, -25, -24, -23, -17, -16, -14, -12, -11, -9, -8, 7, 8, 10, 11, 13, 15, 16, 22, 23, 24, 25, 26, 34, 35, 36, 38, 39, 45, 46, 48, 49, 51, 52, 53, 55, 56, 58, 59, 62, 63, 69, 70};
     static constexpr int16_t dc[nd] = {-1, 1, -1, 1, -1, 1, -1, 1, -1, 1, -1, 1, -1, 1, -1, -1, 1, -1, 1, -1, -1, 1, -1, 1, -1, -1, 1, -1, 1, -1, 1, -1, 1, -1, 1, -1, 1, -1, 1, 1, -1, 1, -1, 1, 1, -1, 1, -1, 1, 1, -1, 1, -1, 1, -1, 1, -1, 1, -1, 1, -1, 1, -1, 1};
+    static constexpr int mixed = 1, ns = 8, nb = 28;
+    static constexpr int16_t se[8] = {-52, -35, -23, -14, 13, 22, 34, 51};
+    static constexpr int16_t sc[8] = {-1, -1, -1, -1, 1, 1, 1, 1};
+    static constexpr int16_t be[28] = {-70, -63, -59, -56, -53, -49, -46, -39, -36, -26, -24, -16, -11, -8, 8, 11, 16, 24, 26, 36, 39, 46, 49, 53, 56, 59, 63, 70};
+    static constexpr int16_t bc[28] = {1, 1, 1, 1, 1, -1, -1, 1, 1, 1, 1, 1, -1, -1, -1, -1, 1, 1, 1, 1, 1, -1, -1, 1, 1, 1, 1, 1};
 };
 
 template <>
@@ -143,6 +223,11 @@
     static constexpr uint16_t w[n] = {1, 0, 0, 0, 0, 0, 0, 0, 0, 1, 0, 0, 0, 0, 1, 0, 0, 0, 1, 0, 0, 1, 0, 1, 0, 0, 1, 0, 1, 1, 0, 1, 1, 0, 1, 1, 1, 1, 1, 1, 1, 1, 1, 1, 1, 2, 1, 2, 1, 2, 1, 2, 1, 2, 2, 2, 2, 2, 2, 2, 2, 2, 3, 2, 3, 2, 2, 3, 3, 2, 3, 3, 3, 2, 3, 3, 3, 3, 3, 3, 3, 4, 3, 3, 3, 3, 3, 3, 4, 3, 3, 3, 3, 3, 3, 4, 3, 3, 3, 3, 3, 3, 3, 2, 3, 3, 3, 2, 3, 3, 2, 2, 3, 2, 3, 2, 2, 2, 2, 2, 2, 2, 2, 2, 1, 2, 1, 2, 1, 2, 1, 2, 1, 1, 1, 1, 1, 1, 1, 1, 1, 1, 1, 0, 1, 1, 0, 1, 1, 0, 1, 0, 0, 1, 0, 1, 0, 0, 1, 0, 0, 0, 1, 0, 0, 0, 0, 1, 0, 0, 0, 0, 0, 0, 0, 0, 1};
     static constexpr int16_t de[nd] = {-89, -88, -80, -79, -75, -74, -71, -70, -68, -67, -66, -65, -63, -62, -61, -59, -58, -56, -55, -44, -43, -42, -41, -40, -39, -38, -37, -36, -27, -26, -25, -24, -22, -20, -19, -16, -15, -8, -7, -1, 0, 6, 7, 14, 15, 18, 19, 21, 23, 24, 25, 26, 35, 36, 37, 38, 39, 40, 41, 42, 43, 54, 55, 57, 58, 60, 61, 62, 64, 65, 66, 67, 69, 70, 73, 74, 78, 79, 87, 88};
     static constexpr int16_t dc[nd] = {-1, 1, -1, 1, -1, 1, -1, 1, -1, 1, -1, 1, -1, 1, -1, 1, -1, 1, -1, -1, 1, -1, 1, -1, 1, -1, 1, -1, -1, 1, -1, 1, -1, 1, -1, 1, -1, -1, 1, -1, 1, -1, 1, 1, -1, 1, -1, 1, -1, 1, -1, 1, 1, -1, 1, -1, 1, -1, 1, -1, 1, 1, -1, 1, -1, 1, -1, 1, -1, 1, -1, 1, -1, 1, -1, 1, -1, 1, -1, 1};
+    static constexpr int mixed = 1, ns = 6, nb = 37;
+    static constexpr int16_t se[6] = {-61, -36, -22, 21, 35, 60};
+    static constexpr int16_t sc[6] = {-1, -1, -1, 1, 1, 1};
+    static constexpr int16_t be[37] = {-88, -79, -74, -70, -67, -65, -62, -58, -55, -43, -41, -39, -37, -26, -24, -19, -15, -7, 0, 7, 15, 19, 24, 26, 37, 39, 41, 43, 55, 58, 62, 65, 67, 70, 74, 79, 88};
+    static constexpr int16_t bc[37] = {1, 1, 1, 1, 1, 1, 1, -1, -1, 1, 1, 1, 1, 1, 1, -1, -1, 1, 1, 1, -1, -1, 1, 1, 1, 1, 1, 1, -1, -1, 1, 1, 1, 1, 1, 1, 1};
 };
 
 template <>
@@ -151,6 +236,11 @@
     static constexpr uint16_t w[n] = {1, 0, 0, 0, 0, 0, 0, 0, 0, 0, 0, 1, 0, 0, 0, 0, 0, 0, 1, 0, 0, 0, 0, 1, 0, 0, 0, 1, 0, 0, 1, 0, 1, 0, 0, 1, 0, 1, 0, 1, 0, 1, 0, 1, 1, 0, 1, 1, 1, 0, 1, 1, 1, 1, 1, 1, 1, 1, 1, 1, 1, 1, 2, 1, 1, 1, 2, 1, 2, 1, 2, 1, 2, 1, 2, 2, 1, 2, 2, 2, 2, 2, 2, 2, 2, 2, 2, 2, 2, 2, 2, 3, 2, 2, 3, 2, 2, 3, 2, 2, 3, 2, 3, 2, 3, 2, 3, 2, 3, 2, 3, 2, 3, 2, 3, 2, 3, 2, 3, 2, 3, 2, 3, 2, 2, 3, 2, 2, 3, 2, 2, 3, 2, 2, 2, 2, 2, 2, 2, 2, 2, 2, 2, 2, 2, 2, 1, 2, 2, 1, 2, 1, 2, 1, 2, 1, 2, 1, 1, 1, 2, 1, 1, 1, 1, 1, 1, 1, 1, 1, 1, 1, 1, 0, 1, 1, 1, 0, 1, 1, 0, 1, 0, 1, 0, 1, 0, 1, 0, 0, 1, 0, 1, 0, 0, 1, 0, 0, 0, 1, 0, 0, 0, 0, 1, 0, 0, 0, 0, 0, 0, 1, 0, 0, 0, 0, 0, 0, 0, 0, 0, 0, 1};
     static constexpr int16_t de[nd] = {-112, -111, -101, -100, -94, -93, -89, -88, -85, -84, -82, -81, -80, -79, -77, -76, -75, -74, -73, -72, -71, -70, -69, -67, -66, -63, -62, -50, -49, -46, -45, -44, -43, -42, -41, -40, -39, -38, -36, -35, -21, -20, -18, -17, -15, -14, -12, -11, -10, -9, -8, -7, -6, -5, -4, -3, -2, -1, 0, 1, 2, 3, 4, 5, 6, 7, 8, 9, 10, 11, 13, 14, 16, 17, 19, 20, 34, 35, 37, 38, 39, 40, 41, 42, 43, 44, 45, 48, 49, 61, 62, 65, 66, 68, 69, 70, 71, 72, 73, 74, 75, 76, 78, 79, 80, 81, 83, 84, 87, 88, 92, 93, 99, 100, 110, 111};
     static constexpr int16_t dc[nd] = {-1, 1, -1, 1, -1, 1, -1, 1, -1, 1, -1, 1, -1, 1, -1, 1, -1, 1, -1, 1, -1, 1, -1, 1, -1, 1, -1, -1, 1, -1, 1, -1, 1, -1, 1, -1, 1, -1, 1, -1, -1, 1, -1, 1, -1, 1, -1, 1, -1, 1, -1, 1, -1, 1, -1, 1, -1, 1, -1, 1, -1, 1, -1, 1, -1, 1, -1, 1, -1, 1, -1, 1, -1, 1, -1, 1, 1, -1, 1, -1, 1, -1, 1, -1, 1, -1, 1, -1, 1, 1, -1, 1, -1, 1, -1, 1, -1, 1, -1, 1, -1, 1, -1, 1, -1, 1, -1, 1, -1, 1, -1, 1, -1, 1, -1, 1};
+    static constexpr int mixed = 1, ns = 4, nb = 56;
+    static constexpr int16_t se[4] = {-69, -38, 37, 68};
+    static constexpr int16_t sc[4] = {-1, -1, 1, 1};
+    static constexpr int16_t be[56] = {-111, -100, -93, -88, -84, -81, -79, -76, -74, -72, -70, -66, -62, -49, -45, -43, -41, -39, -35, -20, -17, -14, -11, -9, -7, -5, -3, -1, 1, 3, 5, 7, 9, 11, 14, 17, 20, 35, 39, 41, 43, 45, 49, 62, 66, 70, 72, 74, 76, 79, 81, 84, 88, 93, 100, 111};
+    static constexpr int16_t bc[56] = {1, 1, 1, 1, 1, 1, 1, 1, 1, 1, 1, -1, -1, 1, 1, 1, 1, 1, -1, 1, 1, 1, 1, 1, 1, 1, 1, 1, 1, 1, 1, 1, 1, 1, 1, 1, 1, -1, 1, 1, 1, 1, 1, -1, -1, 1, 1, 1, 1, 1, 1, 1, 1, 1, 1, 1};
 };
 
 }
diff --git a/visualslam_amd/csrc/kernels_hdiff.hip.h b/visualslam_amd/csrc/kernels_hdiff.hip.h
--- a/visualslam_amd/csrc/kernels_hdiff.hip.h
+++ b/visualslam_amd/csrc/kernels_hdiff.hip.h
@@ -30,7 +30,23 @@
 __host__ __device__ constexpr int hd_w(int k) { return k >= 0 && k < LV::n ? (int)LV::w[k] : 0; }
 
 template <class LV>
+__host__ __device__ constexpr int hd_spike(int e) {
+    if (LV::mixed == 1)
+        for (int i = 0; i < LV::nb; ++i)
+            if (LV::be[i] == e) return LV::bc[i];
+    return 0;
+}
+
+template <class LV>
+__host__ __device__ constexpr int hd_seed_w(int k) { return k >= 0 && k < LV::n ? (int)LV::w[k] - hd_spike<LV>(k - LV::n / 2) : 0; }
+
+template <class LV>
 __host__ __device__ constexpr int hd_coef(int e) {
+    if (LV::mixed == 1) {
+        for (int i = 0; i < LV::ns; ++i)
+            if (LV::se[i] == e) return LV::sc[i];
+        return 0;
+    }
     if (LV::form == 1) {
         for (int i = 0; i < LV::nd; ++i)
             if (LV::de[i] == e) return LV::dc[i];
@@ -55,11 +71,13 @@
 template <class LV, int HL>
 __device__ __forceinline__ void hd_level(const hd_f2* __restrict__ lane, hd_f2 (&acc)[HD_J]) {
     constexpr int n = LV::n, r = n / 2;
-    constexpr bool DIFF = LV::form == 1;
+    constexpr bool MIXED = LV::mixed == 1, DIFF = MIXED || LV::form == 1;
     constexpr int lo = DIFF ? -r - 1 : -r, hi = HD_J - 1 + r;
     constexpr int t0 = (HL + lo) & ~1, Q = (HL + hi - t0) / 2 + 1;
     hd_f2 seed = {0.f, 0.f};
+    hd_f2 dir[MIXED ? HD_J : 1];
     hd_for<HD_J>([&](auto j) { acc[decltype(j)::value] = hd_f2{0.f, 0.f}; });
+    if constexpr (MIXED) hd_for<HD_J>([&](auto j) { dir[decltype(j)::value] = hd_f2{0.f, 0.f}; });
     hd_for<Q>([&](auto q) {
         constexpr int t = t0 + 2 * decltype(q)::value;
         const float4 v = *reinterpret_cast<const float4*>(lane + hd_phys(t));
@@ -67,13 +85,18 @@
         hd_for<2>([&](auto b) {
             constexpr int x = t + decltype(b)::value - HL;
             if constexpr (DIFF) {
-                constexpr int wk = hd_w<LV>(x + 1 + r);
+                constexpr int wk = hd_seed_w<LV>(x + 1 + r);
                 if constexpr (wk != 0) seed = __builtin_elementwise_fma(hd_f2((float)wk), hv[decltype(b)::value], seed);
             }
             hd_for<HD_J>([&](auto j) {
                 constexpr int c = hd_coef<LV>(x - decltype(j)::value);
                 if constexpr (c != 0)
                     acc[decltype(j)::value] = __builtin_elementwise_fma(hd_f2((float)c), hv[decltype(b)::value], acc[decltype(j)::value]);
+                if constexpr (MIXED) {
+                    constexpr int s = hd_spike<LV>(x - decltype(j)::value);
+                    if constexpr (s != 0)
+                        dir[decltype(j)::value] = __builtin_elementwise_fma(hd_f2((float)s), hv[decltype(b)::value], dir[decltype(j)::value]);
+                }
             });
         });
     });
@@ -81,6 +104,7 @@
         acc[0] += seed;
         hd_for<HD_J - 1>([&](auto j) { acc[decltype(j)::value + 1] += acc[decltype(j)::value]; });
     }
+    if constexpr (MIXED) hd_for<HD_J>([&](auto j) { acc[decltype(j)::value] += dir[decltype(j)::value]; });
 }
 
 template <int O>
@@ -175,6 +199,12 @@
         for (int i = 0; i < LV::nd; ++i)
             if (off[i] != LV::de[i] || coef[i] != LV::dc[i]) return false;
     }
+    MixedForm m;
+    if (mixed_form(t.data(), LV::n, m) != LV::mixed || (int)m.s_off.size() != LV::ns || (int)m.b_off.size() != LV::nb) return false;
+    for (int i = 0; i < LV::ns; ++i)
+        if (m.s_off[i] != LV::se[i] || m.s_coef[i] != LV::sc[i]) return false;
+    for (int i = 0; i < LV::nb; ++i)
+        if (m.b_off[i] != LV::be[i] || m.b_coef[i] != LV::bc[i]) return false;
     return true;
 }
 template <int O>
diff --git a/visualslam_amd/csrc/vslam_internal.h b/visualslam_amd/csrc/vslam_internal.h
--- a/visualslam_amd/csrc/vslam_internal.h
+++ b/visualslam_amd/csrc/vslam_internal.h
@@ -19,6 +19,12 @@
 void extrema_lattice(int rows, int cols, int window, int* lr, int* lc);
 int make_layout(const vslam_params* p, vslam_batch_layout* L);
 int diff_form(const uint16_t* w, int n, std::vector<int>& off, std::vector<int>& coef);
+struct MixedForm {
+    std::vector<int> s_off, s_coef, b_off, b_coef;
+};
+int mixed_form(const uint16_t* w, int n, MixedForm& m);
 }
 
 extern "C" int vslam_diff_form_q8(const uint16_t* taps, int n, int* offsets, int* coeffs, int cap, int* nnz);
+extern "C" int vslam_mixed_form_q8(const uint16_t* taps, int n, int* step_offsets, int* step_coeffs, int* n_steps, int* spike_offsets,
+                                   int* spike_coeffs, int* n_spikes, int cap);
diff --git a/visualslam_amd/csrc/vslam_params.cpp b/visualslam_amd/csrc/vslam_params.cpp
--- a/visualslam_amd/csrc/vslam_params.cpp
+++ b/visualslam_amd/csrc/vslam_params.cpp
@@ -92,6 +92,66 @@
     }
     if (l1 * DIFF_HMAX >= (1L << 24)) return 0;
     return (double)off.size() * 2.32 * 1.15 <= (double)(n + 1) / 2 * 4.27 ? 1 : 0;
+}
+
+int mixed_form(const uint16_t* w, int n, MixedForm& m) {
+    m = MixedForm{};
+    if (!w || n <= 0 || (n & 1) == 0) return -1;
+    constexpr int D = 3, NV = 2 * D + 1;
+    const int r = n / 2;
+    const uint64_t INF = ~(uint64_t)0;
+    auto term = [](int u, int v, int wk) {
+        const int a = v > wk ? v - wk : wk - v;
+        return ((uint64_t)(16 * ((u != v) + (v != wk)) + (v != 0)) << 16) + (uint64_t)a;
+    };
+    std::vector<uint64_t> cost((size_t)n * NV, INF);
+    std::vector<int8_t> from((size_t)n * NV, -1);
+    for (int k = 0; k < n; ++k)
+        for (int i = 0; i < NV; ++i) {
+            const int v = (int)w[k] - D + i;
+            if (v < 0) continue;
+            if (k == 0) {
+                cost[(size_t)i] = term(0, v, w[0]);
+                continue;
+            }
+            for (int p = 0; p < NV; ++p) {
+                const uint64_t c0 = cost[(size_t)(k - 1) * NV + p];
+                if (c0 == INF) continue;
+                const uint64_t c = c0 + term((int)w[k - 1] - D + p, v, w[k]);
+                if (c < cost[(size_t)k * NV + i]) cost[(size_t)k * NV + i] = c, from[(size_t)k * NV + i] = (int8_t)p;
+            }
+        }
+    int bi = -1;
+    uint64_t best = INF;
+    for (int i = 0; i < NV; ++i) {
+        const uint64_t c0 = cost[(size_t)(n - 1) * NV + i];
+        if (c0 == INF) continue;
+        const uint64_t c = c0 + ((uint64_t)(16 * ((int)w[n - 1] - D + i != 0)) << 16);
+        if (c < best) best = c, bi = i;
+    }
+    std::vector<int> s((size_t)n);
+    for (int k = n - 1; k >= 0; --k) {
+        s[(size_t)k] = (int)w[k] - D + bi;
+        bi = from[(size_t)k * NV + bi];
+    }
+    long sum_s = 0, l1_ds = 0, l1_b = 0;
+    for (int e = -r - 1; e <= r; ++e) {
+        const int k = e + r;
+        const int d = (k >= 0 ? s[(size_t)k] : 0) - (k + 1 < n ? s[(size_t)k + 1] : 0);
+        if (d) m.s_off.push_back(e), m.s_coef.push_back(d), l1_ds += d < 0 ? -d : d;
+    }
+    for (int k = 0; k < n; ++k) {
+        const int b = (int)w[k] - s[(size_t)k];
+        sum_s += s[(size_t)k];
+        if (b) m.b_off.push_back(k - r), m.b_coef.push_back(b), l1_b += b < 0 ? -b : b;
+    }
+    const long lim = 1L << 24;
+    if (sum_s * DIFF_HMAX >= lim || l1_ds * DIFF_HMAX >= lim || l1_b * DIFF_HMAX >= lim) return 0;
+    const size_t macs = m.s_off.size() + m.b_off.size() + 1;
+    if ((double)macs * 2.32 * 1.15 > (double)(n + 1) / 2 * 4.27) return 0;
+    std::vector<int> off, coef;
+    if (diff_form(w, n, off, coef) == 1 && macs >= off.size()) return 0;
+    return 1;
 }
 
 double sigma_at(double sigma0, int octave, int level) {
@@ -186,6 +246,19 @@
     for (size_t i = 0; i < off.size(); ++i) offsets[i] = off[i], coeffs[i] = coef[i];
     return form;
 }
+
+int vslam_mixed_form_q8(const uint16_t* taps, int n, int* step_offsets, int* step_coeffs, int* n_steps, int* spike_offsets,
+                        int* spike_coeffs, int* n_spikes, int cap) {
+    vslam::MixedForm m;
+    const int mixed = vslam::mixed_form(taps, n, m);
+    if (mixed < 0 || !n_steps || !n_spikes || (int)m.s_off.size() > cap || (int)m.b_off.size() > cap) return -1;
+    if ((!m.s_off.empty() && (!step_offsets || !step_coeffs)) || (!m.b_off.empty() && (!spike_offsets || !spike_coeffs))) return -1;
+    *n_steps = (int)m.s_off.size(), *n_spikes = (int)m.b_off.size();
+    for (size_t i = 0; i < m.s_off.size(); ++i) step_offsets[i] = m.s_off[i], step_coeffs[i] = m.s_coef[i];
+    for (size_t i = 0; i < m.b_off.size(); ++i) spike_offsets[i] = m.b_off[i], spike_coeffs[i] = m.b_coef[i];
+    return mixed;
+}
+
 int vslam_auto_num_octaves(int rows, int cols) { return vslam::auto_num_octaves(rows, cols); }
 
 void vslam_half_size(int rows, int cols, int* out_rows, int* out_cols) {
```

Measured after the change: 15010, median of 6. Within noise of the previous version (+1.0%).
